# nvidia-cosmos/cosmos-curate

Measured on NVIDIA H100. Metric: clips_per_sec, higher is better.
Workload: dtype f16

## Files before the change

### cosmos_curate_b200/csrc/gemm.cu

```cuda
#include <cuda_fp16.h>

#include <algorithm>
#include <cstdlib>

#include "common.h"
#include "ptx.cuh"

namespace cb {

constexpr int BM = 128, BK = 64;
constexpr int kGemmThreads = 384;
constexpr int kEpiRows = 64, kEpiBytes = kEpiRows * 128;

template <int BN>
struct GemmCfg {
  static constexpr int kStages = (BN == 256) ? 4 : 6;
  static constexpr int kABytes = BM * BK * 2, kBBytes = BN * BK * 2;
  static constexpr int kStageBytes = kABytes + kBBytes;
  static constexpr int kRingBytes = kStages * kStageBytes;
  static constexpr int kEpiTotal = 2  * 2  * kEpiBytes;
  static constexpr int kSmem = kRingBytes + kEpiTotal + 1024  + 256 ;
  static_assert(kSmem <= 232448, "over the 227 KB of opt-in shared memory per block on sm_90");
};

struct GemmArgs {
  const float* bias;
  int M, N, K;
  int residual;
  const float* gamma;
};

__device__ __forceinline__ float act_quick_gelu(float x) { return __fdividef(x, 1.f + exp2f(-2.4554669595930156f * x)); }
__device__ __forceinline__ float act_gelu_tanh(float x) {
  const float k0 = 0.7978845608028654f, k1 = 0.044715f;
  const float u = k0 * (x + k1 * x * x * x);
  const float e = exp2f(2.885390081777927f * u);
  const float t = 1.f - __fdividef(2.f, e + 1.f);
  return 0.5f * x * (1.f + t);
}

__device__ __forceinline__ float act_gelu_erf(float x) { return 0.5f * x * (1.f + erff(x * 0.7071067811865476f)); }

template <int ACT>
__device__ __forceinline__ float act(float x) {
  if (ACT == CB_EPI_QUICK_GELU) return act_quick_gelu(x);
  if (ACT == CB_EPI_GELU_TANH) return act_gelu_tanh(x);
  if (ACT == CB_EPI_GELU_ERF) return act_gelu_erf(x);
  return x;
}

template <int BN>
__device__ __forceinline__ void wgmma_tile(float* d, uint64_t da, uint64_t db, int accumulate) {
  if (BN == 256) wgmma_m64n256k16(d, da, db, accumulate);
  else wgmma_m64n128k16(d, da, db, accumulate);
}

template <int BN, int ACT, bool OUT_F32, bool SCALE = false>
__global__ void __launch_bounds__(kGemmThreads, 1)
    gemm_wgmma_kernel(const __grid_constant__ CUtensorMap map_a, const __grid_constant__ CUtensorMap map_b, const __grid_constant__ CUtensorMap map_o,
                      const __grid_constant__ CUtensorMap map_r, const GemmArgs g) {
  using Cfg = GemmCfg<BN>;
  constexpr int kSliceCols = OUT_F32 ? 32 : 64;
  constexpr int kSlices = BN / kSliceCols;
  constexpr int kSliceJ = kSliceCols / 8;
  extern __shared__ __align__(1024) uint8_t smem_raw[];
  const uint32_t base = (smem_u32(smem_raw) + 1023u) & ~1023u;
  uint8_t* smem = smem_raw + (base - smem_u32(smem_raw));
  uint8_t* sA = smem;
  uint8_t* sB = smem + Cfg::kStages * Cfg::kABytes;
  uint8_t* sE = smem + Cfg::kRingBytes;
  uint64_t* full = (uint64_t*)(smem + Cfg::kRingBytes + Cfg::kEpiTotal);
  uint64_t* empty = full + Cfg::kStages;
  uint64_t* rfull = empty + Cfg::kStages;

  const int warp = threadIdx.x >> 5, lane = threadIdx.x & 31, wg = warp >> 2;
  const int m_tiles = (g.M + BM - 1) / BM, n_tiles = (g.N + BN - 1) / BN;
  const int num_tiles = m_tiles * n_tiles;
  const int num_kb = (g.K + BK - 1) / BK;
  const int first = blockIdx.x, step = gridDim.x;
  const bool has_res = OUT_F32 && g.residual;

  if (threadIdx.x == 0) {
    tma_prefetch_desc(&map_a);
    tma_prefetch_desc(&map_b);
    tma_prefetch_desc(&map_o);
    if (has_res) tma_prefetch_desc(&map_r);
    for (int i = 0; i < Cfg::kStages; ++i) {
      mbar_init(&full[i], 1);
      mbar_init(&empty[i], 2);
    }
    for (int i = 0; i < 4; ++i) mbar_init(&rfull[i], 1);
    fence_barrier_init();
  }
  __syncthreads();

  if (wg == 0) {
    reg_dealloc<40>();
    if (warp == 0 && lane == 0) {
      int stage = 0;
      uint32_t phase = 0;
      for (int t = first; t < num_tiles; t += step) {
        const int m_blk = t / n_tiles, n_blk = t % n_tiles;
        if (has_res)
          for (int r = 0; r < BM; r += kEpiRows)
            for (int cc = 0; cc < BN && n_blk * BN + cc < g.N; cc += kSliceCols) tma_prefetch_l2_2d(&map_r, n_blk * BN + cc, m_blk * BM + r);
        for (int kb = 0; kb < num_kb; ++kb) {
          mbar_wait(&empty[stage], phase ^ 1);
          mbar_expect_tx(&full[stage], Cfg::kStageBytes);
          tma_load_2d(sA + stage * Cfg::kABytes, &map_a, &full[stage], kb * BK, m_blk * BM);
          tma_load_2d(sB + stage * Cfg::kBBytes, &map_b, &full[stage], kb * BK, n_blk * BN);
          if (++stage == Cfg::kStages) stage = 0, phase ^= 1;
        }
      }
    }
  } else {
    reg_alloc<232>();
    const int c = wg - 1;
    const bool leader = (threadIdx.x & 127) == 0;
    auto release = [&](int s) {
      if (leader) mbar_arrive(&empty[s]);
    };
    uint8_t* ebuf = sE + c * 2 * kEpiBytes;
    uint64_t* rbar = rfull + 2 * c;
    int eb = 0;
    uint32_t rphase = 0;
    int stage = 0;
    uint32_t phase = 0;
    float acc[BN / 2];
    float2 bias[BN / 8];
    float2 gam[SCALE ? BN / 8 : 1];
    for (int t = first; t < num_tiles; t += step) {
      const int m_blk = t / n_tiles, n_blk = t % n_tiles;
      const int row0 = m_blk * BM + c * 64, col0 = n_blk * BN;
      const int nslices = row0 >= g.M ? 0 : std::min(kSlices, (g.N - col0 + kSliceCols - 1) / kSliceCols);
      int prev = -1;
      for (int kb = 0; kb < num_kb; ++kb) {
        mbar_wait(&full[stage], phase);
        const uint64_t da = wgmma_desc_sw128(smem_u32(sA + stage * Cfg::kABytes + c * (64 * 128)));
        const uint64_t db = wgmma_desc_sw128(smem_u32(sB + stage * Cfg::kBBytes));
        wgmma_fence();
#pragma unroll
        for (int k = 0; k < BK / 16; ++k) wgmma_tile<BN>(acc, da + (uint64_t)(2 * k), db + (uint64_t)(2 * k), (kb | k) != 0);
        wgmma_commit();
        if (kb == 0 && has_res && leader) {
          bulk_wait_read<0>();
          for (int s = 0; s < 2 && s < nslices; ++s) {
            const int b = eb ^ s;
            mbar_expect_tx(&rbar[b], kEpiBytes);
            tma_load_2d(ebuf + b * kEpiBytes, &map_r, &rbar[b], col0 + s * kSliceCols, row0);
          }
        }
        wgmma_wait<1>();
        if (prev >= 0) release(prev);
        prev = stage;
        if (++stage == Cfg::kStages) stage = 0, phase ^= 1;
      }
#pragma unroll
      for (int j = 0; j < BN / 8; ++j) {
        const int col = col0 + 8 * j + 2 * (lane & 3);
        bias[j] = (g.bias && col < g.N) ? __ldg((const float2*)(g.bias + col)) : make_float2(0.f, 0.f);
        if (SCALE) gam[j] = col < g.N ? __ldg((const float2*)(g.gamma + col)) : make_float2(0.f, 0.f);
      }
      wgmma_wait<0>();
      release(prev);

      const int rl = (warp & 3) * 16 + (lane >> 2), sw = lane >> 2;
#pragma unroll
      for (int s = 0; s < kSlices; ++s) {
        if (s >= nslices) break;
        uint8_t* buf = ebuf + eb * kEpiBytes;
        if (has_res) {
          mbar_wait(&rbar[eb], (rphase >> eb) & 1);
          rphase ^= 1u << eb;
        } else {
          if (leader) bulk_wait_read<1>();
          named_bar_sync(1 + c, 128);
        }
#pragma unroll
        for (int jj = 0; jj < kSliceJ; ++jj) {
          const int j = s * kSliceJ + jj;
#pragma unroll
          for (int h = 0; h < 2; ++h) {
            uint8_t* row = buf + (rl + 8 * h) * 128;
            float v0 = act<ACT>(acc[4 * j + 2 * h] + bias[j].x), v1 = act<ACT>(acc[4 * j + 2 * h + 1] + bias[j].y);
            if (SCALE) v0 = __fmul_rn(v0, gam[j].x), v1 = __fmul_rn(v1, gam[j].y);
            if (OUT_F32) {
              float2* p = (float2*)(row + (((2 * jj + ((lane & 3) >> 1)) ^ sw) << 4) + 8 * (lane & 1));
              if (has_res) {
                const float2 rr = *p;
                v0 += rr.x, v1 += rr.y;
              }
              *p = make_float2(v0, v1);
            } else {
              *(__half2*)(row + ((jj ^ sw) << 4) + 4 * (lane & 3)) = __floats2half2_rn(v0, v1);
            }
          }
        }
        fence_proxy_async();
        named_bar_sync(1 + c, 128);
        if (leader) {
          tma_store_2d(&map_o, buf, col0 + s * kSliceCols, row0);
          bulk_commit();
          if (has_res && s + 2 < nslices) {
            bulk_wait_read<0>();
            mbar_expect_tx(&rbar[eb], kEpiBytes);
            tma_load_2d(buf, &map_r, &rbar[eb], col0 + (s + 2) * kSliceCols, row0);
          }
        }
        eb ^= 1;
      }
    }
    if (leader) bulk_wait<0>();
  }
}

template <int BN, int ACT, bool OUT_F32, bool SCALE = false>
static int launch_gemm(cb_ctx* ctx, const CUtensorMap& ma, const CUtensorMap& mb, const CUtensorMap& mo, const CUtensorMap& mr, const GemmArgs& g,
                       cudaStream_t stream) {
  using Cfg = GemmCfg<BN>;
  auto kern = gemm_wgmma_kernel<BN, ACT, OUT_F32, SCALE>;
  static bool attr_done[64] = {};
  bool& attr_set = attr_done[ctx->device & 63];
  if (!attr_set) {
    CB_CUDA(ctx, cudaFuncSetAttribute(kern, cudaFuncAttributeMaxDynamicSharedMemorySize, Cfg::kSmem));
    attr_set = true;
  }
  const int tiles = ((g.M + BM - 1) / BM) * ((g.N + BN - 1) / BN);
  mark_launch(ctx, CB_PROF_GEMM, stream);
  kern<<<std::min(tiles, ctx->sm_count), kGemmThreads, Cfg::kSmem, stream>>>(ma, mb, mo, mr, g);
  CB_CUDA(ctx, cudaGetLastError());
  return CB_OK;
}

template <int BN>
static int dispatch_gemm(cb_ctx* ctx, const CUtensorMap& ma, const CUtensorMap& mb, const CUtensorMap& mo, const CUtensorMap& mr, const GemmArgs& g,
                         bool out_f32, int epilogue, cudaStream_t stream) {
  if (out_f32) return launch_gemm<BN, CB_EPI_NONE, true>(ctx, ma, mb, mo, mr, g, stream);
  if (epilogue == CB_EPI_QUICK_GELU) return launch_gemm<BN, CB_EPI_QUICK_GELU, false>(ctx, ma, mb, mo, mr, g, stream);
  if (epilogue == CB_EPI_GELU_TANH) return launch_gemm<BN, CB_EPI_GELU_TANH, false>(ctx, ma, mb, mo, mr, g, stream);
  if (epilogue == CB_EPI_GELU_ERF) return launch_gemm<BN, CB_EPI_GELU_ERF, false>(ctx, ma, mb, mo, mr, g, stream);
  if (epilogue == CB_EPI_NONE) return launch_gemm<BN, CB_EPI_NONE, false>(ctx, ma, mb, mo, mr, g, stream);
  return fail(ctx, CB_ERR_ARG, "gemm: unknown epilogue %d", epilogue);
}

int gemm_f16_ex(cb_ctx* ctx, const void* A, const void* W, const float* bias, const float* gamma, const float* residual, float* out_f32,
                void* out_f16, int M, int N, int K, int epilogue, cudaStream_t stream) {
  if (!A || !W || (!out_f32 && !out_f16)) return fail(ctx, CB_ERR_ARG, "gemm: null operand");
  if (M <= 0 || N <= 0 || K <= 0) return fail(ctx, CB_ERR_ARG, "gemm: bad shape %dx%dx%d", M, N, K);
  if ((K & 7) || (N & 7)) return fail(ctx, CB_ERR_ARG, "gemm: N and K must be multiples of 8 (got N=%d K=%d)", N, K);
  if (((uintptr_t)A | (uintptr_t)W) & 15) return fail(ctx, CB_ERR_ARG, "gemm: operands must be 16-byte aligned");
  const void* out = out_f32 ? (const void*)out_f32 : out_f16;
  if (((uintptr_t)out | (uintptr_t)residual) & 15) return fail(ctx, CB_ERR_ARG, "gemm: output and residual must be 16-byte aligned");
  if (out_f32 && epilogue != CB_EPI_NONE) return fail(ctx, CB_ERR_UNSUPPORTED, "gemm: activation with fp32 output");
  if (residual && !out_f32) return fail(ctx, CB_ERR_UNSUPPORTED, "gemm: residual needs the fp32 output");
  if (gamma && !out_f32) return fail(ctx, CB_ERR_UNSUPPORTED, "gemm: gamma needs the fp32 output");
  if ((uintptr_t)gamma & 7) return fail(ctx, CB_ERR_ARG, "gemm: gamma must be 8-byte aligned");
  const int tiles256 = ((M + BM - 1) / BM) * ((N + 255) / 256);
  const bool wide = !gamma && (N % 256 == 0 || N > 1024) && tiles256 >= ctx->sm_count;
  const int BN = wide ? 256 : 128;
  CUtensorMap ma, mb, mo, mr;
  uint64_t da[2] = {(uint64_t)K, (uint64_t)M}, db[2] = {(uint64_t)K, (uint64_t)N}, st[1] = {(uint64_t)K * 2};
  uint32_t ba[2] = {BK, BM}, bb[2] = {BK, (uint32_t)BN};
  int rc = make_tensor_map(ctx, &ma, CU_TENSOR_MAP_DATA_TYPE_FLOAT16, 2, A, da, st, ba, CU_TENSOR_MAP_SWIZZLE_128B);
  if (rc) return rc;
  rc = make_tensor_map(ctx, &mb, CU_TENSOR_MAP_DATA_TYPE_FLOAT16, 2, W, db, st, bb, CU_TENSOR_MAP_SWIZZLE_128B);
  if (rc) return rc;
  const uint64_t esz = out_f32 ? 4 : 2;
  uint64_t dout[2] = {(uint64_t)N, (uint64_t)M}, sout[1] = {(uint64_t)N * esz};
  uint32_t bout[2] = {(uint32_t)(128 / esz), (uint32_t)kEpiRows};
  const CUtensorMapDataType dt = out_f32 ? CU_TENSOR_MAP_DATA_TYPE_FLOAT32 : CU_TENSOR_MAP_DATA_TYPE_FLOAT16;
  rc = make_tensor_map(ctx, &mo, dt, 2, out, dout, sout, bout, CU_TENSOR_MAP_SWIZZLE_128B);
  if (rc) return rc;
  mr = mo;
  if (residual && (rc = make_tensor_map(ctx, &mr, dt, 2, residual, dout, sout, bout, CU_TENSOR_MAP_SWIZZLE_128B))) return rc;
  GemmArgs g{bias, M, N, K, residual != nullptr, gamma};
  if (gamma) return launch_gemm<128, CB_EPI_NONE, true, true>(ctx, ma, mb, mo, mr, g, stream);
  return BN == 256 ? dispatch_gemm<256>(ctx, ma, mb, mo, mr, g, out_f32 != nullptr, epilogue, stream)
                   : dispatch_gemm<128>(ctx, ma, mb, mo, mr, g, out_f32 != nullptr, epilogue, stream);
}

int gemm_f16(cb_ctx* ctx, const void* A, const void* W, const float* bias, const float* residual, float* out_f32, void* out_f16, int M,
             int N, int K, int epilogue, cudaStream_t stream) {
  return gemm_f16_ex(ctx, A, W, bias, nullptr, residual, out_f32, out_f16, M, N, K, epilogue, stream);
}

}

extern "C" int cb_gemm_f16_ex(cb_ctx* ctx, const void* A, const void* W, const float* bias, const float* gamma, const float* residual,
                              float* out_f32, void* out_f16, int M, int N, int K, int epilogue, void* stream) {
  if (!ctx) return CB_ERR_ARG;
  return cb::gemm_f16_ex(ctx, A, W, bias, gamma, residual, out_f32, out_f16, M, N, K, epilogue, (cudaStream_t)stream);
}

extern "C" int cb_gemm_f16(cb_ctx* ctx, const void* A, const void* W, const float* bias, const float* residual, float* out_f32,
                           void* out_f16, int M, int N, int K, int epilogue, void* stream) {
  if (!ctx) return CB_ERR_ARG;
  return cb::gemm_f16(ctx, A, W, bias, residual, out_f32, out_f16, M, N, K, epilogue, (cudaStream_t)stream);
}
```

### cosmos_curate_b200/csrc/ptx.cuh

```cuda
#pragma once
#include <cuda.h>
#include <cuda_fp16.h>
#include <stdint.h>

namespace cb {

__device__ __forceinline__ uint32_t smem_u32(const void* p) { return (uint32_t)__cvta_generic_to_shared(p); }

__device__ __forceinline__ void mbar_init(uint64_t* bar, uint32_t count) {
  asm volatile("mbarrier.init.shared::cta.b64 [%0], %1;" ::"r"(smem_u32(bar)), "r"(count));
}
__device__ __forceinline__ void fence_barrier_init() { asm volatile("fence.mbarrier_init.release.cluster;" ::: "memory"); }
__device__ __forceinline__ void fence_proxy_async() { asm volatile("fence.proxy.async.shared::cta;" ::: "memory"); }
__device__ __forceinline__ void mbar_expect_tx(uint64_t* bar, uint32_t bytes) {
  asm volatile("mbarrier.arrive.expect_tx.shared::cta.b64 _, [%0], %1;" ::"r"(smem_u32(bar)), "r"(bytes) : "memory");
}
__device__ __forceinline__ void mbar_arrive(uint64_t* bar) {
  asm volatile("mbarrier.arrive.shared::cta.b64 _, [%0];" ::"r"(smem_u32(bar)) : "memory");
}
__device__ __forceinline__ bool mbar_try_wait(uint64_t* bar, uint32_t parity) {
  uint32_t ok;
  asm volatile(
      "{\n\t.reg .pred p;\n\t"
      "mbarrier.try_wait.parity.shared::cta.b64 p, [%1], %2;\n\t"
// ... 29 lines not shown
        : "r"(smem_u32(bar)), "r"(parity), "r"(ns)
        : "memory");
  } while (!ok);
}

__device__ __forceinline__ void tma_prefetch_desc(const CUtensorMap* m) {
  asm volatile("prefetch.tensormap [%0];" ::"l"(m) : "memory");
}
__device__ __forceinline__ void tma_load_2d(void* dst, const CUtensorMap* m, uint64_t* bar, int c0, int c1) {
  asm volatile(
      "cp.async.bulk.tensor.2d.shared::cluster.global.mbarrier::complete_tx::bytes [%0], [%1, {%3, %4}], [%2];" ::"r"(smem_u32(dst)),
      "l"(m), "r"(smem_u32(bar)), "r"(c0), "r"(c1)
      : "memory");
}
__device__ __forceinline__ void tma_load_3d(void* dst, const CUtensorMap* m, uint64_t* bar, int c0, int c1, int c2) {
  asm volatile(
      "cp.async.bulk.tensor.3d.shared::cluster.global.mbarrier::complete_tx::bytes [%0], [%1, {%3, %4, %5}], [%2];" ::"r"(
          smem_u32(dst)),
      "l"(m), "r"(smem_u32(bar)), "r"(c0), "r"(c1), "r"(c2)
      : "memory");
}
__device__ __forceinline__ void tma_load_5d(void* dst, const CUtensorMap* m, uint64_t* bar, int c0, int c1, int c2, int c3, int c4) {
  asm volatile(
      "cp.async.bulk.tensor.5d.shared::cluster.global.mbarrier::complete_tx::bytes [%0], [%1, {%3, %4, %5, %6, %7}], [%2];" ::"r"(
          smem_u32(dst)),
      "l"(m), "r"(smem_u32(bar)), "r"(c0), "r"(c1), "r"(c2), "r"(c3), "r"(c4)
      : "memory");
}
__device__ __forceinline__ void tma_load_2d_hint(void* dst, const CUtensorMap* m, uint64_t* bar, int c0, int c1, uint64_t policy) {
  asm volatile(
      "cp.async.bulk.tensor.2d.shared::cluster.global.mbarrier::complete_tx::bytes.L2::cache_hint [%0], [%1, {%3, %4}], [%2], %5;" ::"r"(
          smem_u32(dst)),
      "l"(m), "r"(smem_u32(bar)), "r"(c0), "r"(c1), "l"(policy)
      : "memory");
}
__device__ __forceinline__ void tma_prefetch_l2_2d(const CUtensorMap* m, int c0, int c1) {
  asm volatile("cp.async.bulk.prefetch.tensor.2d.L2.global.tile [%0, {%1, %2}];" ::"l"(m), "r"(c0), "r"(c1) : "memory");
}

__device__ __forceinline__ void tma_store_2d(const CUtensorMap* m, const void* src, int c0, int c1) {
  asm volatile("cp.async.bulk.tensor.2d.global.shared::cta.bulk_group [%0, {%2, %3}], [%1];" ::"l"(m), "r"(smem_u32(src)), "r"(c0), "r"(c1)
               : "memory");
}
__device__ __forceinline__ void bulk_commit() { asm volatile("cp.async.bulk.commit_group;" ::: "memory"); }
template <int N>
__device__ __forceinline__ void bulk_wait_read() {
  asm volatile("cp.async.bulk.wait_group.read %0;" ::"n"(N) : "memory");
}
template <int N>
__device__ __forceinline__ void bulk_wait() {
  asm volatile("cp.async.bulk.wait_group %0;" ::"n"(N) : "memory");
}
__device__ __forceinline__ void named_bar_sync(int id, int threads) { asm volatile("bar.sync %0, %1;" ::"r"(id), "r"(threads) : "memory"); }

__device__ __forceinline__ uint64_t policy_evict_first() {
  uint64_t p;
  asm volatile("createpolicy.fractional.L2::evict_first.b64 %0, 1.0;" : "=l"(p));
  return p;
}
__device__ __forceinline__ uint64_t policy_evict_last() {
  uint64_t p;
  asm volatile("createpolicy.fractional.L2::evict_last.b64 %0, 1.0;" : "=l"(p));
  return p;
}
__device__ __forceinline__ void wgmma_fence() { asm volatile("wgmma.fence.sync.aligned;" ::: "memory"); }
__device__ __forceinline__ void wgmma_commit() { asm volatile("wgmma.commit_group.sync.aligned;" ::: "memory"); }
template <int N>
__device__ __forceinline__ void wgmma_wait() {
  asm volatile("wgmma.wait_group.sync.aligned %0;" ::"n"(N) : "memory");
}
template <int REGS>
__device__ __forceinline__ void reg_alloc() { asm volatile("setmaxnreg.inc.sync.aligned.u32 %0;" ::"n"(REGS)); }
template <int REGS>
__device__ __forceinline__ void reg_dealloc() { asm volatile("setmaxnreg.dec.sync.aligned.u32 %0;" ::"n"(REGS)); }
// ... 52 lines not shown
        "+f"(d[56]), "+f"(d[57]), "+f"(d[58]), "+f"(d[59]), "+f"(d[60]), "+f"(d[61]), "+f"(d[62]), "+f"(d[63]),
        "+f"(d[64]), "+f"(d[65]), "+f"(d[66]), "+f"(d[67]), "+f"(d[68]), "+f"(d[69]), "+f"(d[70]), "+f"(d[71]),
        "+f"(d[72]), "+f"(d[73]), "+f"(d[74]), "+f"(d[75]), "+f"(d[76]), "+f"(d[77]), "+f"(d[78]), "+f"(d[79]),
        "+f"(d[80]), "+f"(d[81]), "+f"(d[82]), "+f"(d[83]), "+f"(d[84]), "+f"(d[85]), "+f"(d[86]), "+f"(d[87]),
        "+f"(d[88]), "+f"(d[89]), "+f"(d[90]), "+f"(d[91]), "+f"(d[92]), "+f"(d[93]), "+f"(d[94]), "+f"(d[95]),
        "+f"(d[96]), "+f"(d[97]), "+f"(d[98]), "+f"(d[99]), "+f"(d[100]), "+f"(d[101]), "+f"(d[102]), "+f"(d[103]),
        "+f"(d[104]), "+f"(d[105]), "+f"(d[106]), "+f"(d[107]), "+f"(d[108]), "+f"(d[109]), "+f"(d[110]), "+f"(d[111]),
        "+f"(d[112]), "+f"(d[113]), "+f"(d[114]), "+f"(d[115]), "+f"(d[116]), "+f"(d[117]), "+f"(d[118]), "+f"(d[119]),
        "+f"(d[120]), "+f"(d[121]), "+f"(d[122]), "+f"(d[123]), "+f"(d[124]), "+f"(d[125]), "+f"(d[126]), "+f"(d[127])
      : "l"(desc_a), "l"(desc_b), "r"(accumulate));
}
__device__ __forceinline__ void wgmma_m64n64k16_ra_tb(float* d, const uint32_t* a, uint64_t desc_b, int accumulate) {
  asm volatile(
      "{\n\t.reg .pred p;\n\tsetp.ne.b32 p, %37, 0;\n\t"
      "wgmma.mma_async.sync.aligned.m64n64k16.f32.f16.f16 {%0, %1, %2, %3, %4, %5, %6, %7, %8, %9, %10, %11, %12, %13, %14, %15, %16, %17, %18, %19, %20, %21, %22, %23, %24, %25, %26, %27, %28, %29, %30, %31}, {%32, %33, %34, %35}, %36, p, 1, 1, 1;\n\t}"
      :
        "+f"(d[0]), "+f"(d[1]), "+f"(d[2]), "+f"(d[3]), "+f"(d[4]), "+f"(d[5]), "+f"(d[6]), "+f"(d[7]),
        "+f"(d[8]), "+f"(d[9]), "+f"(d[10]), "+f"(d[11]), "+f"(d[12]), "+f"(d[13]), "+f"(d[14]), "+f"(d[15]),
        "+f"(d[16]), "+f"(d[17]), "+f"(d[18]), "+f"(d[19]), "+f"(d[20]), "+f"(d[21]), "+f"(d[22]), "+f"(d[23]),
        "+f"(d[24]), "+f"(d[25]), "+f"(d[26]), "+f"(d[27]), "+f"(d[28]), "+f"(d[29]), "+f"(d[30]), "+f"(d[31])
      : "r"(a[0]), "r"(a[1]), "r"(a[2]), "r"(a[3]), "l"(desc_b), "r"(accumulate));
}

__device__ __forceinline__ uint32_t cluster_ctarank() {
  uint32_t r;
  asm volatile("mov.u32 %0, %%cluster_ctarank;" : "=r"(r));
  return r;
}
__device__ __forceinline__ void cluster_sync_all() {
  asm volatile("barrier.cluster.arrive.release.aligned;" ::: "memory");
  asm volatile("barrier.cluster.wait.acquire.aligned;" ::: "memory");
}
__device__ __forceinline__ void mbar_arrive_cluster(uint32_t addr) {
  asm volatile("mbarrier.arrive.release.cluster.shared::cluster.b64 _, [%0];" ::"r"(addr) : "memory");
}
__device__ __forceinline__ uint32_t map_to_cta(const void* local, uint32_t rank) {
  uint32_t r;
  asm volatile("mapa.shared::cluster.u32 %0, %1, %2;" : "=r"(r) : "r"(smem_u32(local)), "r"(rank));
  return r;
}

}
```

### cosmos_curate_b200/_lib.py

```python

from __future__ import annotations

import ctypes as C
import os
from pathlib import Path

PKG = Path(__file__).resolve().parent
LIB_PATH = PKG / "libcurate_b200.so"

CB_OK = 0
CB_ERR = {-1: "CB_ERR_CUDA", -2: "CB_ERR_ARG", -3: "CB_ERR_UNSUPPORTED", -4: "CB_ERR_NVDEC", -5: "CB_ERR_DEMUX", -6: "CB_ERR_STATE", -7: "CB_ERR_INVALID"}
ROWDOT_UPPER, ROWDOT_CLIP = 1, 2
FMT_NV12, FMT_RGB24, FMT_NV12_SWS = 0, 1, 2
DT_F16, DT_BF16, DT_F32 = 0, 1, 2
LAYOUT_NCHW, LAYOUT_PATCH = 0, 1
ACT_QUICK_GELU, ACT_GELU_TANH = 0, 1
ARCH_CLIP, ARCH_SIGLIP = 0, 1
EPI_NONE, EPI_QUICK_GELU, EPI_GELU_TANH, EPI_GELU_ERF = 0, 1, 2, 3
DECODE_SEEK_SYNC, DECODE_DISCARD_ALL = 1, 2
CUBIC_OPENCV, CUBIC_IPP = 0, 1


class CurateB200Error(RuntimeError):
    def __init__(self, code: int, where: str, msg: str):
# ... 63 lines not shown
    "cb_video_tube": (_i, [_vp, C.POINTER(SurfacePool), _pi32, _i, _i, _i, _pf, _pf, _vp, _vp, _vp]),
    "cb_video_tube_patches": (_i, [_vp, C.POINTER(SurfacePool), _pi32, _i, _i, _i, _i, _pf, _pf, _vp, _vp]),
    "cb_nv12_to_rgb": (_i, [_vp, C.POINTER(SurfacePool), _pi32, _i, _vp, _vp]),
    "cb_vit_create": (_i, [_vp, C.POINTER(VitCfg), C.POINTER(_vp)]),
    "cb_vit_destroy": (None, [_vp]),
    "cb_vit_set_tensor": (_i, [_vp, C.c_char_p, _pf, C.c_size_t]),
    "cb_vit_set_aesthetic": (_i, [_vp, _pf, C.c_size_t, _f]),
    "cb_vit_finalize": (_i, [_vp, _i]),
    "cb_vit_k_pad": (_i, [_vp]),
    "cb_vit_forward": (_i, [_vp, _vp, _i, _vp, _vp, _vp, _vp]),
    "cb_vit_embed_surfaces": (_i, [_vp, C.POINTER(SurfacePool), _pi32, _i, _pf, _pf, _vp, _vp, _vp, _vp]),
    "cb_affine_score": (_i, [_vp, _vp, _vp, _f, _vp, _i, _i, _vp]),
    "cb_mp4_index": (_i, [_vp, _vp, C.c_size_t, C.POINTER(Mp4Info), C.POINTER(C.c_int64), C.POINTER(C.c_uint8), _i]),
    "cb_mp4_cut": (_i, [_vp, _vp, C.c_size_t, _i, _i, _vp, C.c_size_t, C.POINTER(C.c_size_t)]),
    "cb_nvdec_probe": (_i, [_vp]),
    "cb_decoder_create": (_i, [_vp, C.POINTER(_vp)]),
    "cb_decoder_destroy": (None, [_vp]),
    "cb_decoder_decode": (_i, [_vp, _vp, C.c_size_t, _pi32, _i, C.POINTER(SurfacePool), _pi32, C.POINTER(DecodeStats)]),
    "cb_decoder_decode_ex": (_i, [_vp, _vp, C.c_size_t, _pi32, _i, C.POINTER(SurfacePool), _pi32, _i, C.POINTER(DecodeStats)]),
    "cb_decoder_decode_thumbnails": (_i, [_vp, _vp, C.c_size_t, _i, _i, _vp, _i, C.POINTER(DecodeStats)]),
    "cb_transnet_create": (_i, [_vp, C.POINTER(_vp)]),
    "cb_transnet_destroy": (None, [_vp]),
    "cb_transnet_set_tensor": (_i, [_vp, C.c_char_p, _vp, C.c_size_t]),
    "cb_transnet_finalize": (_i, [_vp, _i]),
    "cb_transnet_forward": (_i, [_vp, _vp, _i, _i, _vp, _vp]),
    "cb_transnet_predict": (_i, [_vp, _vp, _i, _vp, _vp]),
    "cb_rowdot_argmax": (_i, [_vp, _vp, _i, _vp, _i, _i, _vp, _i, _f, _vp, _vp, _vp]),
    "cb_rows_l2_normalize": (_i, [_vp, _vp, _i, _i, _vp, _vp]),
    "cb_cluster_sums": (_i, [_vp, _vp, _vp, _vp, _i, _i, _vp, _vp]),
    "cb_gemm_f16": (_i, [_vp, _vp, _vp, _vp, _vp, _vp, _vp, _i, _i, _i, _i, _vp]),
    "cb_layernorm_f16": (_i, [_vp, _vp, _vp, _vp, _vp, _i, _i, _f, _vp]),
    "cb_attention_f16": (_i, [_vp, _vp, _vp, _i, _i, _i, _i, _vp]),
    "cb_gemm_f16_ex": (_i, [_vp, _vp, _vp, _vp, _vp, _vp, _vp, _vp, _i, _i, _i, _i, _vp]),
    "cb_rmsnorm_f16": (_i, [_vp, _vp, _vp, _vp, _i, _i, _f, _vp]),
    "cb_qk_rmsnorm_f16": (_i, [_vp, _vp, _vp, _vp, _i, _i, _f, _vp]),
    "cb_attention_stream_f16": (_i, [_vp, _vp, _vp, _i, _i, _i, _i, _vp]),
    "cb_iv2_create": (_i, [_vp, C.POINTER(Iv2Cfg), C.POINTER(_vp)]),
    "cb_iv2_destroy": (None, [_vp]),
    "cb_iv2_set_tensor": (_i, [_vp, C.c_char_p, _pf, C.c_size_t]),
    "cb_iv2_finalize": (_i, [_vp, _i]),
    "cb_iv2_forward": (_i, [_vp, _vp, _i, _vp, _vp]),
    "cb_iv2_embed_surfaces": (_i, [_vp, C.POINTER(SurfacePool), _pi32, _i, _pf, _pf, _vp, _vp]),
    "cb_attention_masked_f16": (_i, [_vp, _vp, _vp, _i, _i, _i, _i, _vp, _vp]),
    "cb_layernorm_post_f16": (_i, [_vp, _vp, _vp, _vp, _vp, _i, _i, _f, _vp]),
    "cb_text_embed": (_i, [_vp, _vp, _vp, _vp, _vp, _vp, _i, _i, _i, _vp]),
    "cb_assemble_tokens": (_i, [_vp, _vp, _vp, _vp, _vp, _vp, _vp, _i, _i, _i, _i, _f, _vp]),
    "cb_clip_tail": (_i, [_vp, _vp, C.c_size_t, _vp, _vp, _vp, _i, _i, _f, _vp, _f, _vp, _vp, _vp, _i, _vp]),
    "cb_map_pool": (_i, [_vp, _vp, _vp, _vp, _i, _i, _i, _i, _vp]),
    "cb_l2norm_score": (_i, [_vp, _vp, _i, _vp, _f, _vp, _vp, _vp, _i, _vp]),
    "cb_token_mean": (_i, [_vp, _vp, _vp, _i, _i, _i, _vp]),
    "cb_clip_pool": (_i, [_vp, _vp, _vp, _vp, _vp, _i, _i, _i, _i, _vp]),
    "cb_tube_patches": (_i, [_vp, _vp, _vp, _i, _i, _i, _i, _vp]),
    "cb_iv2_text_create": (_i, [_vp, C.POINTER(Iv2TextCfg), C.POINTER(_vp)]),
    "cb_iv2_text_destroy": (None, [_vp]),
    "cb_iv2_text_set_tensor": (_i, [_vp, C.c_char_p, _pf, C.c_size_t]),
    "cb_iv2_text_finalize": (_i, [_vp, _i, _i]),
    "cb_iv2_text_forward": (_i, [_vp, _pi32, _pi32, _i, _i, _vp, _vp]),
}

_lib = None


def header_symbols() -> list[str]:
    import re

    text = (PKG.parent / "include" / "curate_b200.h").read_text()
# ... 23 lines not shown
```

### include/curate_b200.h

```cpp
#ifndef CURATE_B200_H
#define CURATE_B200_H

#include <stddef.h>
#include <stdint.h>

#ifdef __cplusplus
extern "C" {
#endif

#define CB_OK 0
#define CB_ERR_CUDA (-1)
#define CB_ERR_ARG (-2)
#define CB_ERR_UNSUPPORTED (-3)
#define CB_ERR_NVDEC (-4)
#define CB_ERR_DEMUX (-5)
#define CB_ERR_STATE (-6)
#define CB_ERR_INVALID (-7)

#define CB_ABI_VERSION 1

typedef struct cb_ctx cb_ctx;
typedef struct cb_vit cb_vit;

int cb_abi_version(void);
// ... 109 lines not shown
#define CB_DECODE_DISCARD_ALL 2
int cb_decoder_decode_ex(cb_decoder* dec, const uint8_t* data, size_t size, const int32_t* frame_ids, int n_ids,
                         const cb_surface_pool* dst, const int32_t* dst_slots, int flags, cb_decode_stats* stats);

int cb_decoder_decode_thumbnails(cb_decoder* dec, const uint8_t* data, size_t size, int out_w, int out_h, uint8_t* out,
                                 int max_frames, cb_decode_stats* stats);

typedef struct cb_transnet cb_transnet;
int cb_transnet_create(cb_ctx* ctx, cb_transnet** out);
void cb_transnet_destroy(cb_transnet* tn);
int cb_transnet_set_tensor(cb_transnet* tn, const char* name, const float* data, size_t count);
int cb_transnet_finalize(cb_transnet* tn, int max_windows);
int cb_transnet_forward(cb_transnet* tn, const uint8_t* windows, int n_windows, int frames_per_window, float* prob_out, void* stream);
int cb_transnet_predict(cb_transnet* tn, const uint8_t* frames, int n_frames, float* prob_out, void* stream);

#define CB_ROWDOT_UPPER 1
#define CB_ROWDOT_CLIP 2
int cb_rowdot_argmax(cb_ctx* ctx, const float* a, int na, const float* b, int nb, int d, const float* bias, int flags, float init_val, float* out_val,
                     int* out_idx, void* stream);
int cb_rows_l2_normalize(cb_ctx* ctx, float* x, int rows, int d, float* norms_out, void* stream);
int cb_cluster_sums(cb_ctx* ctx, const float* x, const long long* order, const long long* seg, int n_clusters, int d, float* sums, void* stream);

#define CB_EPI_NONE 0
#define CB_EPI_QUICK_GELU 1
#define CB_EPI_GELU_TANH 2
#define CB_EPI_GELU_ERF 3
int cb_gemm_f16(cb_ctx* ctx, const void* A, const void* W, const float* bias, const float* residual, float* out_f32,
                void* out_f16, int M, int N, int K, int epilogue, void* stream);
int cb_layernorm_f16(cb_ctx* ctx, const float* x, const float* gamma, const float* beta, void* y, int rows, int d, float eps,
                     void* stream);
int cb_attention_f16(cb_ctx* ctx, const void* qkv, void* out, int n, int tokens, int heads, int head_dim, void* stream);
int cb_gemm_f16_ex(cb_ctx* ctx, const void* A, const void* W, const float* bias, const float* gamma, const float* residual, float* out_f32,
                   void* out_f16, int M, int N, int K, int epilogue, void* stream);
int cb_rmsnorm_f16(cb_ctx* ctx, const float* x, const float* weight, void* y, int rows, int d, float eps, void* stream);
int cb_qk_rmsnorm_f16(cb_ctx* ctx, void* qkv, const float* q_weight, const float* k_weight, int rows, int d, float eps, void* stream);
int cb_attention_stream_f16(cb_ctx* ctx, const void* qkv, void* out, int n, int tokens, int heads, int head_dim, void* stream);
int cb_attention_masked_f16(cb_ctx* ctx, const void* qkv, void* out, int n, int tokens, int heads, int head_dim, const int* lengths, void* stream);
int cb_layernorm_post_f16(cb_ctx* ctx, float* h, const float* gamma, const float* beta, void* y, int rows, int d, float eps, void* stream);
int cb_text_embed(cb_ctx* ctx, const int32_t* ids, const float* word, const float* pos, const float* type, float* h, int n, int L, int d,
                  void* stream);
int cb_assemble_tokens(cb_ctx* ctx, const float* patch, const float* cls, const float* pos, const float* gamma, const float* beta, float* h, int n,
                       int tokens, int grid2, int d, float eps, void* stream);
int cb_clip_tail(cb_ctx* ctx, const float* h, size_t img_stride, const float* gamma, const float* beta, const float* proj, int d, int proj_dim,
                 float eps, const float* aes_w, float aes_b, float* emb_out, float* feat_out, float* score_out, int n, void* stream);
int cb_map_pool(cb_ctx* ctx, const void* kv, const float* q, void* out, int n, int tokens, int heads, int head_dim, void* stream);
int cb_l2norm_score(cb_ctx* ctx, const float* feat, int d, const float* aes_w, float aes_b, float* emb_out, float* feat_out, float* score_out, int n,
                    void* stream);
int cb_token_mean(cb_ctx* ctx, const float* h, float* out, int n, int tokens, int d, void* stream);
int cb_clip_pool(cb_ctx* ctx, const float* q, const void* k, const void* v, void* out, int n, int tokens, int heads, int head_dim, void* stream);
int cb_tube_patches(cb_ctx* ctx, const float* tubes, void* out, int frames, int image_size, int patch, int k_pad, void* stream);

typedef struct cb_iv2 cb_iv2;
typedef struct cb_iv2_cfg {
  int image_size, patch, frames;
  int hidden, layers, heads, mlp;
  int clip_dim, embed_dim;
  float rms_eps, ln_eps;
} cb_iv2_cfg;
int cb_iv2_create(cb_ctx* ctx, const cb_iv2_cfg* cfg, cb_iv2** out);
void cb_iv2_destroy(cb_iv2* iv2);
int cb_iv2_set_tensor(cb_iv2* iv2, const char* name, const float* data, size_t count);
int cb_iv2_finalize(cb_iv2* iv2, int max_clips);
int cb_iv2_forward(cb_iv2* iv2, const float* tubes, int n, float* emb_out, void* stream);
int cb_iv2_embed_surfaces(cb_iv2* iv2, const cb_surface_pool* pool, const int32_t* slots, int n_clips, const float mean[3], const float std_[3],
                          float* emb_out, void* stream);

// ... 17 lines not shown
```

Measured before the change: 264.1.

## Fuse residual add into TMA reduce-add store instead of loading residual tiles

Drops the residual TMA loads, L2 prefetches and the extra mbarriers from the GEMM epilogue. The f32 output tile is now written with a TMA bulk reduce-add into the output buffer, which is pre-filled with the residual by a device-to-device memcpy when the two buffers differ. This simplifies the epilogue pipeline and removes a synchronisation dependency on residual loads. In exchange it may add a full memcpy of the residual, and a reduce-add read-modify-write in L2, whenever residual is not aliased with the output.

```diff
diff --git a/cosmos_curate_b200/csrc/gemm.cu b/cosmos_curate_b200/csrc/gemm.cu
--- a/cosmos_curate_b200/csrc/gemm.cu
+++ b/cosmos_curate_b200/csrc/gemm.cu
@@ -58,7 +58,7 @@
 template <int BN, int ACT, bool OUT_F32, bool SCALE = false>
 __global__ void __launch_bounds__(kGemmThreads, 1)
     gemm_wgmma_kernel(const __grid_constant__ CUtensorMap map_a, const __grid_constant__ CUtensorMap map_b, const __grid_constant__ CUtensorMap map_o,
-                      const __grid_constant__ CUtensorMap map_r, const GemmArgs g) {
+                      const GemmArgs g) {
   using Cfg = GemmCfg<BN>;
   constexpr int kSliceCols = OUT_F32 ? 32 : 64;
   constexpr int kSlices = BN / kSliceCols;
@@ -71,7 +71,6 @@
   uint8_t* sE = smem + Cfg::kRingBytes;
   uint64_t* full = (uint64_t*)(smem + Cfg::kRingBytes + Cfg::kEpiTotal);
   uint64_t* empty = full + Cfg::kStages;
-  uint64_t* rfull = empty + Cfg::kStages;
 
   const int warp = threadIdx.x >> 5, lane = threadIdx.x & 31, wg = warp >> 2;
   const int m_tiles = (g.M + BM - 1) / BM, n_tiles = (g.N + BN - 1) / BN;
@@ -84,12 +83,10 @@
     tma_prefetch_desc(&map_a);
     tma_prefetch_desc(&map_b);
     tma_prefetch_desc(&map_o);
-    if (has_res) tma_prefetch_desc(&map_r);
     for (int i = 0; i < Cfg::kStages; ++i) {
       mbar_init(&full[i], 1);
       mbar_init(&empty[i], 2);
     }
-    for (int i = 0; i < 4; ++i) mbar_init(&rfull[i], 1);
     fence_barrier_init();
   }
   __syncthreads();
@@ -101,9 +98,6 @@
       uint32_t phase = 0;
       for (int t = first; t < num_tiles; t += step) {
         const int m_blk = t / n_tiles, n_blk = t % n_tiles;
-        if (has_res)
-          for (int r = 0; r < BM; r += kEpiRows)
-            for (int cc = 0; cc < BN && n_blk * BN + cc < g.N; cc += kSliceCols) tma_prefetch_l2_2d(&map_r, n_blk * BN + cc, m_blk * BM + r);
         for (int kb = 0; kb < num_kb; ++kb) {
           mbar_wait(&empty[stage], phase ^ 1);
           mbar_expect_tx(&full[stage], Cfg::kStageBytes);
@@ -121,9 +115,7 @@
       if (leader) mbar_arrive(&empty[s]);
     };
     uint8_t* ebuf = sE + c * 2 * kEpiBytes;
-    uint64_t* rbar = rfull + 2 * c;
     int eb = 0;
-    uint32_t rphase = 0;
     int stage = 0;
     uint32_t phase = 0;
     float acc[BN / 2];
@@ -142,14 +134,6 @@
 #pragma unroll
         for (int k = 0; k < BK / 16; ++k) wgmma_tile<BN>(acc, da + (uint64_t)(2 * k), db + (uint64_t)(2 * k), (kb | k) != 0);
         wgmma_commit();
-        if (kb == 0 && has_res && leader) {
-          bulk_wait_read<0>();
-          for (int s = 0; s < 2 && s < nslices; ++s) {
-            const int b = eb ^ s;
-            mbar_expect_tx(&rbar[b], kEpiBytes);
-            tma_load_2d(ebuf + b * kEpiBytes, &map_r, &rbar[b], col0 + s * kSliceCols, row0);
-          }
-        }
         wgmma_wait<1>();
         if (prev >= 0) release(prev);
         prev = stage;
@@ -169,13 +153,8 @@
       for (int s = 0; s < kSlices; ++s) {
         if (s >= nslices) break;
         uint8_t* buf = ebuf + eb * kEpiBytes;
-        if (has_res) {
-          mbar_wait(&rbar[eb], (rphase >> eb) & 1);
-          rphase ^= 1u << eb;
-        } else {
-          if (leader) bulk_wait_read<1>();
-          named_bar_sync(1 + c, 128);
-        }
+        if (leader) bulk_wait_read<1>();
+        named_bar_sync(1 + c, 128);
 #pragma unroll
         for (int jj = 0; jj < kSliceJ; ++jj) {
           const int j = s * kSliceJ + jj;
@@ -185,12 +164,7 @@
             float v0 = act<ACT>(acc[4 * j + 2 * h] + bias[j].x), v1 = act<ACT>(acc[4 * j + 2 * h + 1] + bias[j].y);
             if (SCALE) v0 = __fmul_rn(v0, gam[j].x), v1 = __fmul_rn(v1, gam[j].y);
             if (OUT_F32) {
-              float2* p = (float2*)(row + (((2 * jj + ((lane & 3) >> 1)) ^ sw) << 4) + 8 * (lane & 1));
-              if (has_res) {
-                const float2 rr = *p;
-                v0 += rr.x, v1 += rr.y;
-              }
-              *p = make_float2(v0, v1);
+              *(float2*)(row + (((2 * jj + ((lane & 3) >> 1)) ^ sw) << 4) + 8 * (lane & 1)) = make_float2(v0, v1);
             } else {
               *(__half2*)(row + ((jj ^ sw) << 4) + 4 * (lane & 3)) = __floats2half2_rn(v0, v1);
             }
@@ -199,13 +173,9 @@
         fence_proxy_async();
         named_bar_sync(1 + c, 128);
         if (leader) {
-          tma_store_2d(&map_o, buf, col0 + s * kSliceCols, row0);
+          if (has_res) tma_reduce_add_2d(&map_o, buf, col0 + s * kSliceCols, row0);
+          else tma_store_2d(&map_o, buf, col0 + s * kSliceCols, row0);
           bulk_commit();
-          if (has_res && s + 2 < nslices) {
-            bulk_wait_read<0>();
-            mbar_expect_tx(&rbar[eb], kEpiBytes);
-            tma_load_2d(buf, &map_r, &rbar[eb], col0 + (s + 2) * kSliceCols, row0);
-          }
         }
         eb ^= 1;
       }
@@ -215,7 +185,7 @@
 }
 
 template <int BN, int ACT, bool OUT_F32, bool SCALE = false>
-static int launch_gemm(cb_ctx* ctx, const CUtensorMap& ma, const CUtensorMap& mb, const CUtensorMap& mo, const CUtensorMap& mr, const GemmArgs& g,
+static int launch_gemm(cb_ctx* ctx, const CUtensorMap& ma, const CUtensorMap& mb, const CUtensorMap& mo, const GemmArgs& g,
                        cudaStream_t stream) {
   using Cfg = GemmCfg<BN>;
   auto kern = gemm_wgmma_kernel<BN, ACT, OUT_F32, SCALE>;
@@ -227,19 +197,19 @@
   }
   const int tiles = ((g.M + BM - 1) / BM) * ((g.N + BN - 1) / BN);
   mark_launch(ctx, CB_PROF_GEMM, stream);
-  kern<<<std::min(tiles, ctx->sm_count), kGemmThreads, Cfg::kSmem, stream>>>(ma, mb, mo, mr, g);
+  kern<<<std::min(tiles, ctx->sm_count), kGemmThreads, Cfg::kSmem, stream>>>(ma, mb, mo, g);
   CB_CUDA(ctx, cudaGetLastError());
   return CB_OK;
 }
 
 template <int BN>
-static int dispatch_gemm(cb_ctx* ctx, const CUtensorMap& ma, const CUtensorMap& mb, const CUtensorMap& mo, const CUtensorMap& mr, const GemmArgs& g,
+static int dispatch_gemm(cb_ctx* ctx, const CUtensorMap& ma, const CUtensorMap& mb, const CUtensorMap& mo, const GemmArgs& g,
                          bool out_f32, int epilogue, cudaStream_t stream) {
-  if (out_f32) return launch_gemm<BN, CB_EPI_NONE, true>(ctx, ma, mb, mo, mr, g, stream);
-  if (epilogue == CB_EPI_QUICK_GELU) return launch_gemm<BN, CB_EPI_QUICK_GELU, false>(ctx, ma, mb, mo, mr, g, stream);
-  if (epilogue == CB_EPI_GELU_TANH) return launch_gemm<BN, CB_EPI_GELU_TANH, false>(ctx, ma, mb, mo, mr, g, stream);
-  if (epilogue == CB_EPI_GELU_ERF) return launch_gemm<BN, CB_EPI_GELU_ERF, false>(ctx, ma, mb, mo, mr, g, stream);
-  if (epilogue == CB_EPI_NONE) return launch_gemm<BN, CB_EPI_NONE, false>(ctx, ma, mb, mo, mr, g, stream);
+  if (out_f32) return launch_gemm<BN, CB_EPI_NONE, true>(ctx, ma, mb, mo, g, stream);
+  if (epilogue == CB_EPI_QUICK_GELU) return launch_gemm<BN, CB_EPI_QUICK_GELU, false>(ctx, ma, mb, mo, g, stream);
+  if (epilogue == CB_EPI_GELU_TANH) return launch_gemm<BN, CB_EPI_GELU_TANH, false>(ctx, ma, mb, mo, g, stream);
+  if (epilogue == CB_EPI_GELU_ERF) return launch_gemm<BN, CB_EPI_GELU_ERF, false>(ctx, ma, mb, mo, g, stream);
+  if (epilogue == CB_EPI_NONE) return launch_gemm<BN, CB_EPI_NONE, false>(ctx, ma, mb, mo, g, stream);
   return fail(ctx, CB_ERR_ARG, "gemm: unknown epilogue %d", epilogue);
 }
 
@@ -258,7 +228,7 @@
   const int tiles256 = ((M + BM - 1) / BM) * ((N + 255) / 256);
   const bool wide = !gamma && (N % 256 == 0 || N > 1024) && tiles256 >= ctx->sm_count;
   const int BN = wide ? 256 : 128;
-  CUtensorMap ma, mb, mo, mr;
+  CUtensorMap ma, mb, mo;
   uint64_t da[2] = {(uint64_t)K, (uint64_t)M}, db[2] = {(uint64_t)K, (uint64_t)N}, st[1] = {(uint64_t)K * 2};
   uint32_t ba[2] = {BK, BM}, bb[2] = {BK, (uint32_t)BN};
   int rc = make_tensor_map(ctx, &ma, CU_TENSOR_MAP_DATA_TYPE_FLOAT16, 2, A, da, st, ba, CU_TENSOR_MAP_SWIZZLE_128B);
@@ -271,12 +241,11 @@
   const CUtensorMapDataType dt = out_f32 ? CU_TENSOR_MAP_DATA_TYPE_FLOAT32 : CU_TENSOR_MAP_DATA_TYPE_FLOAT16;
   rc = make_tensor_map(ctx, &mo, dt, 2, out, dout, sout, bout, CU_TENSOR_MAP_SWIZZLE_128B);
   if (rc) return rc;
-  mr = mo;
-  if (residual && (rc = make_tensor_map(ctx, &mr, dt, 2, residual, dout, sout, bout, CU_TENSOR_MAP_SWIZZLE_128B))) return rc;
+  if (residual && residual != out_f32) CB_CUDA(ctx, cudaMemcpyAsync(out_f32, residual, (size_t)M * N * sizeof(float), cudaMemcpyDeviceToDevice, stream));
   GemmArgs g{bias, M, N, K, residual != nullptr, gamma};
-  if (gamma) return launch_gemm<128, CB_EPI_NONE, true, true>(ctx, ma, mb, mo, mr, g, stream);
-  return BN == 256 ? dispatch_gemm<256>(ctx, ma, mb, mo, mr, g, out_f32 != nullptr, epilogue, stream)
-                   : dispatch_gemm<128>(ctx, ma, mb, mo, mr, g, out_f32 != nullptr, epilogue, stream);
+  if (gamma) return launch_gemm<128, CB_EPI_NONE, true, true>(ctx, ma, mb, mo, g, stream);
+  return BN == 256 ? dispatch_gemm<256>(ctx, ma, mb, mo, g, out_f32 != nullptr, epilogue, stream)
+                   : dispatch_gemm<128>(ctx, ma, mb, mo, g, out_f32 != nullptr, epilogue, stream);
 }
 
 int gemm_f16(cb_ctx* ctx, const void* A, const void* W, const float* bias, const float* residual, float* out_f32, void* out_f16, int M,
diff --git a/cosmos_curate_b200/csrc/ptx.cuh b/cosmos_curate_b200/csrc/ptx.cuh
--- a/cosmos_curate_b200/csrc/ptx.cuh
+++ b/cosmos_curate_b200/csrc/ptx.cuh
@@ -87,12 +87,14 @@
       "l"(m), "r"(smem_u32(bar)), "r"(c0), "r"(c1), "l"(policy)
       : "memory");
 }
-__device__ __forceinline__ void tma_prefetch_l2_2d(const CUtensorMap* m, int c0, int c1) {
-  asm volatile("cp.async.bulk.prefetch.tensor.2d.L2.global.tile [%0, {%1, %2}];" ::"l"(m), "r"(c0), "r"(c1) : "memory");
-}
 
 __device__ __forceinline__ void tma_store_2d(const CUtensorMap* m, const void* src, int c0, int c1) {
   asm volatile("cp.async.bulk.tensor.2d.global.shared::cta.bulk_group [%0, {%2, %3}], [%1];" ::"l"(m), "r"(smem_u32(src)), "r"(c0), "r"(c1)
+               : "memory");
+}
+__device__ __forceinline__ void tma_reduce_add_2d(const CUtensorMap* m, const void* src, int c0, int c1) {
+  asm volatile("cp.reduce.async.bulk.tensor.2d.global.shared::cta.add.tile.bulk_group [%0, {%2, %3}], [%1];" ::"l"(m), "r"(smem_u32(src)),
+               "r"(c0), "r"(c1)
                : "memory");
 }
 __device__ __forceinline__ void bulk_commit() { asm volatile("cp.async.bulk.commit_group;" ::: "memory"); }
```

After: 270.8, median of 6. +2.5%, better.

## Pair BN=256 GEMM CTAs into 2-CTA clusters with multicast weight loads

Applied to the files above, without the earlier changes.

For the wide (BN=256) GEMM, CTAs are launched in 2-CTA clusters that work on adjacent M tiles sharing the same N tile. Each CTA loads half of the weight tile and multicasts it to both CTAs, so weight traffic from L2 is cut in half. Empty barriers now expect arrivals from both CTAs' consumers, and cluster syncs are added at start and end. The risks are cluster scheduling constraints, an error return when the grid is odd, extra cross-CTA synchronisation, and the removal of release semantics from the cluster arrive.

```diff
diff --git a/cosmos_curate_b200/_lib.py b/cosmos_curate_b200/_lib.py
--- a/cosmos_curate_b200/_lib.py
+++ b/cosmos_curate_b200/_lib.py
@@ -119,6 +119,7 @@
     "cb_layernorm_f16": (_i, [_vp, _vp, _vp, _vp, _vp, _i, _i, _f, _vp]),
     "cb_attention_f16": (_i, [_vp, _vp, _vp, _i, _i, _i, _i, _vp]),
     "cb_gemm_f16_ex": (_i, [_vp, _vp, _vp, _vp, _vp, _vp, _vp, _vp, _i, _i, _i, _i, _vp]),
+    "cb_gemm_pair_clusters": (_i, [_vp, _vp]),
     "cb_rmsnorm_f16": (_i, [_vp, _vp, _vp, _vp, _i, _i, _f, _vp]),
     "cb_qk_rmsnorm_f16": (_i, [_vp, _vp, _vp, _vp, _i, _i, _f, _vp]),
     "cb_attention_stream_f16": (_i, [_vp, _vp, _vp, _i, _i, _i, _i, _vp]),
diff --git a/cosmos_curate_b200/csrc/gemm.cu b/cosmos_curate_b200/csrc/gemm.cu
--- a/cosmos_curate_b200/csrc/gemm.cu
+++ b/cosmos_curate_b200/csrc/gemm.cu
@@ -12,8 +12,11 @@
 constexpr int kGemmThreads = 384;
 constexpr int kEpiRows = 64, kEpiBytes = kEpiRows * 128;
 
+constexpr int kWBoxRows = 128;
+
 template <int BN>
 struct GemmCfg {
+  static constexpr int kPair = BN == 256 ? 2 : 1;
   static constexpr int kStages = (BN == 256) ? 4 : 6;
   static constexpr int kABytes = BM * BK * 2, kBBytes = BN * BK * 2;
   static constexpr int kStageBytes = kABytes + kBBytes;
@@ -60,6 +63,7 @@
     gemm_wgmma_kernel(const __grid_constant__ CUtensorMap map_a, const __grid_constant__ CUtensorMap map_b, const __grid_constant__ CUtensorMap map_o,
                       const __grid_constant__ CUtensorMap map_r, const GemmArgs g) {
   using Cfg = GemmCfg<BN>;
+  constexpr int kPair = Cfg::kPair;
   constexpr int kSliceCols = OUT_F32 ? 32 : 64;
   constexpr int kSlices = BN / kSliceCols;
   constexpr int kSliceJ = kSliceCols / 8;
@@ -75,9 +79,10 @@
 
   const int warp = threadIdx.x >> 5, lane = threadIdx.x & 31, wg = warp >> 2;
   const int m_tiles = (g.M + BM - 1) / BM, n_tiles = (g.N + BN - 1) / BN;
-  const int num_tiles = m_tiles * n_tiles;
+  const int rank = kPair == 2 ? (int)cluster_ctarank() : 0;
+  const int num_units = (m_tiles + kPair - 1) / kPair * n_tiles;
   const int num_kb = (g.K + BK - 1) / BK;
-  const int first = blockIdx.x, step = gridDim.x;
+  const int first = blockIdx.x / kPair, step = gridDim.x / kPair;
   const bool has_res = OUT_F32 && g.residual;
 
   if (threadIdx.x == 0) {
@@ -87,28 +92,33 @@
     if (has_res) tma_prefetch_desc(&map_r);
     for (int i = 0; i < Cfg::kStages; ++i) {
       mbar_init(&full[i], 1);
-      mbar_init(&empty[i], 2);
+      mbar_init(&empty[i], 2 * kPair);
     }
     for (int i = 0; i < 4; ++i) mbar_init(&rfull[i], 1);
     fence_barrier_init();
   }
-  __syncthreads();
+  if (kPair == 2) cluster_sync_all();
+  else __syncthreads();
 
   if (wg == 0) {
     reg_dealloc<40>();
     if (warp == 0 && lane == 0) {
       int stage = 0;
       uint32_t phase = 0;
-      for (int t = first; t < num_tiles; t += step) {
-        const int m_blk = t / n_tiles, n_blk = t % n_tiles;
-        if (has_res)
+      for (int u = first; u < num_units; u += step) {
+        const int m_blk = u / n_tiles * kPair + rank, n_blk = u % n_tiles;
+        if (has_res && m_blk < m_tiles)
           for (int r = 0; r < BM; r += kEpiRows)
             for (int cc = 0; cc < BN && n_blk * BN + cc < g.N; cc += kSliceCols) tma_prefetch_l2_2d(&map_r, n_blk * BN + cc, m_blk * BM + r);
         for (int kb = 0; kb < num_kb; ++kb) {
           mbar_wait(&empty[stage], phase ^ 1);
           mbar_expect_tx(&full[stage], Cfg::kStageBytes);
           tma_load_2d(sA + stage * Cfg::kABytes, &map_a, &full[stage], kb * BK, m_blk * BM);
-          tma_load_2d(sB + stage * Cfg::kBBytes, &map_b, &full[stage], kb * BK, n_blk * BN);
+          uint8_t* b = sB + stage * Cfg::kBBytes;
+          if (kPair == 2)
+            tma_load_2d_multicast(b + rank * kWBoxRows * 128, &map_b, &full[stage], kb * BK, n_blk * BN + rank * kWBoxRows, 0x3);
+          else
+            tma_load_2d(b, &map_b, &full[stage], kb * BK, n_blk * BN);
           if (++stage == Cfg::kStages) stage = 0, phase ^= 1;
         }
       }
@@ -118,7 +128,13 @@
     const int c = wg - 1;
     const bool leader = (threadIdx.x & 127) == 0;
     auto release = [&](int s) {
-      if (leader) mbar_arrive(&empty[s]);
+      if (!leader) return;
+      if (kPair == 2) {
+        mbar_arrive_cluster(map_to_cta(&empty[s], 0));
+        mbar_arrive_cluster(map_to_cta(&empty[s], 1));
+      } else {
+        mbar_arrive(&empty[s]);
+      }
     };
     uint8_t* ebuf = sE + c * 2 * kEpiBytes;
     uint64_t* rbar = rfull + 2 * c;
@@ -129,8 +145,8 @@
     float acc[BN / 2];
     float2 bias[BN / 8];
     float2 gam[SCALE ? BN / 8 : 1];
-    for (int t = first; t < num_tiles; t += step) {
-      const int m_blk = t / n_tiles, n_blk = t % n_tiles;
+    for (int u = first; u < num_units; u += step) {
+      const int m_blk = u / n_tiles * kPair + rank, n_blk = u % n_tiles;
       const int row0 = m_blk * BM + c * 64, col0 = n_blk * BN;
       const int nslices = row0 >= g.M ? 0 : std::min(kSlices, (g.N - col0 + kSliceCols - 1) / kSliceCols);
       int prev = -1;
@@ -212,6 +228,16 @@
     }
     if (leader) bulk_wait<0>();
   }
+  if (kPair == 2) {
+    __syncwarp();
+    cluster_sync_all();
+  }
+}
+
+static void set_pair_cluster(cudaLaunchConfig_t& cfg, cudaLaunchAttribute* attr) {
+  attr->id = cudaLaunchAttributeClusterDimension;
+  attr->val.clusterDim.x = 2, attr->val.clusterDim.y = 1, attr->val.clusterDim.z = 1;
+  cfg.attrs = attr, cfg.numAttrs = 1;
 }
 
 template <int BN, int ACT, bool OUT_F32, bool SCALE = false>
@@ -226,8 +252,19 @@
     attr_set = true;
   }
   const int tiles = ((g.M + BM - 1) / BM) * ((g.N + BN - 1) / BN);
-  mark_launch(ctx, CB_PROF_GEMM, stream);
-  kern<<<std::min(tiles, ctx->sm_count), kGemmThreads, Cfg::kSmem, stream>>>(ma, mb, mo, mr, g);
+  if constexpr (Cfg::kPair == 2) {
+    const int grid = std::min(tiles, ctx->sm_count);
+    if (grid & 1) return fail(ctx, CB_ERR_UNSUPPORTED, "gemm: %d CTAs do not pair up into 2-CTA clusters", grid);
+    cudaLaunchConfig_t cfg = {};
+    cudaLaunchAttribute attr;
+    cfg.gridDim = dim3(grid), cfg.blockDim = dim3(kGemmThreads), cfg.dynamicSmemBytes = Cfg::kSmem, cfg.stream = stream;
+    set_pair_cluster(cfg, &attr);
+    mark_launch(ctx, CB_PROF_GEMM, stream);
+    CB_CUDA(ctx, cudaLaunchKernelEx(&cfg, kern, ma, mb, mo, mr, g));
+  } else {
+    mark_launch(ctx, CB_PROF_GEMM, stream);
+    kern<<<std::min(tiles, ctx->sm_count), kGemmThreads, Cfg::kSmem, stream>>>(ma, mb, mo, mr, g);
+  }
   CB_CUDA(ctx, cudaGetLastError());
   return CB_OK;
 }
@@ -260,7 +297,7 @@
   const int BN = wide ? 256 : 128;
   CUtensorMap ma, mb, mo, mr;
   uint64_t da[2] = {(uint64_t)K, (uint64_t)M}, db[2] = {(uint64_t)K, (uint64_t)N}, st[1] = {(uint64_t)K * 2};
-  uint32_t ba[2] = {BK, BM}, bb[2] = {BK, (uint32_t)BN};
+  uint32_t ba[2] = {BK, BM}, bb[2] = {BK, kWBoxRows};
   int rc = make_tensor_map(ctx, &ma, CU_TENSOR_MAP_DATA_TYPE_FLOAT16, 2, A, da, st, ba, CU_TENSOR_MAP_SWIZZLE_128B);
   if (rc) return rc;
   rc = make_tensor_map(ctx, &mb, CU_TENSOR_MAP_DATA_TYPE_FLOAT16, 2, W, db, st, bb, CU_TENSOR_MAP_SWIZZLE_128B);
@@ -284,6 +321,23 @@
   return gemm_f16_ex(ctx, A, W, bias, nullptr, residual, out_f32, out_f16, M, N, K, epilogue, stream);
 }
 
+int gemm_pair_clusters(cb_ctx* ctx, int* clusters) {
+  if (!clusters) return fail(ctx, CB_ERR_ARG, "gemm_pair_clusters: null output");
+  auto kern = gemm_wgmma_kernel<256, CB_EPI_NONE, false>;
+  CB_CUDA(ctx, cudaFuncSetAttribute(kern, cudaFuncAttributeMaxDynamicSharedMemorySize, GemmCfg<256>::kSmem));
+  cudaLaunchConfig_t cfg = {};
+  cudaLaunchAttribute attr;
+  cfg.gridDim = dim3(ctx->sm_count & ~1), cfg.blockDim = dim3(kGemmThreads), cfg.dynamicSmemBytes = GemmCfg<256>::kSmem;
+  set_pair_cluster(cfg, &attr);
+  CB_CUDA(ctx, cudaOccupancyMaxActiveClusters(clusters, kern, &cfg));
+  return CB_OK;
+}
+
+}
+
+extern "C" int cb_gemm_pair_clusters(cb_ctx* ctx, int* clusters) {
+  if (!ctx) return CB_ERR_ARG;
+  return cb::gemm_pair_clusters(ctx, clusters);
 }
 
 extern "C" int cb_gemm_f16_ex(cb_ctx* ctx, const void* A, const void* W, const float* bias, const float* gamma, const float* residual,
diff --git a/cosmos_curate_b200/csrc/ptx.cuh b/cosmos_curate_b200/csrc/ptx.cuh
--- a/cosmos_curate_b200/csrc/ptx.cuh
+++ b/cosmos_curate_b200/csrc/ptx.cuh
@@ -85,6 +85,13 @@
       "cp.async.bulk.tensor.2d.shared::cluster.global.mbarrier::complete_tx::bytes.L2::cache_hint [%0], [%1, {%3, %4}], [%2], %5;" ::"r"(
           smem_u32(dst)),
       "l"(m), "r"(smem_u32(bar)), "r"(c0), "r"(c1), "l"(policy)
+      : "memory");
+}
+__device__ __forceinline__ void tma_load_2d_multicast(void* dst, const CUtensorMap* m, uint64_t* bar, int c0, int c1, uint16_t cta_mask) {
+  asm volatile(
+      "cp.async.bulk.tensor.2d.shared::cluster.global.mbarrier::complete_tx::bytes.multicast::cluster [%0], [%1, {%3, %4}], [%2], %5;" ::"r"(
+          smem_u32(dst)),
+      "l"(m), "r"(smem_u32(bar)), "r"(c0), "r"(c1), "h"(cta_mask)
       : "memory");
 }
 __device__ __forceinline__ void tma_prefetch_l2_2d(const CUtensorMap* m, int c0, int c1) {
@@ -211,7 +218,7 @@
   asm volatile("barrier.cluster.wait.acquire.aligned;" ::: "memory");
 }
 __device__ __forceinline__ void mbar_arrive_cluster(uint32_t addr) {
-  asm volatile("mbarrier.arrive.release.cluster.shared::cluster.b64 _, [%0];" ::"r"(addr) : "memory");
+  asm volatile("mbarrier.arrive.shared::cluster.b64 _, [%0];" ::"r"(addr) : "memory");
 }
 __device__ __forceinline__ uint32_t map_to_cta(const void* local, uint32_t rank) {
   uint32_t r;
diff --git a/include/curate_b200.h b/include/curate_b200.h
--- a/include/curate_b200.h
+++ b/include/curate_b200.h
@@ -165,6 +165,7 @@
 int cb_attention_f16(cb_ctx* ctx, const void* qkv, void* out, int n, int tokens, int heads, int head_dim, void* stream);
 int cb_gemm_f16_ex(cb_ctx* ctx, const void* A, const void* W, const float* bias, const float* gamma, const float* residual, float* out_f32,
                    void* out_f16, int M, int N, int K, int epilogue, void* stream);
+int cb_gemm_pair_clusters(cb_ctx* ctx, int* clusters);
 int cb_rmsnorm_f16(cb_ctx* ctx, const float* x, const float* weight, void* y, int rows, int d, float eps, void* stream);
 int cb_qk_rmsnorm_f16(cb_ctx* ctx, void* qkv, const float* q_weight, const float* k_weight, int rows, int d, float eps, void* stream);
 int cb_attention_stream_f16(cb_ctx* ctx, const void* qkv, void* out, int n, int tokens, int heads, int head_dim, void* stream);
```

Result: no change. 265.1 before, 266.6 after (median of 6 runs) (+0.6%).
